# onolab-tmu/overiva

Measured on AMD Instinct MI355X. Metric: AuxIVA iterations/sec (2048 bins x 4000 frames x 8 mics), higher is better.
Workload: dtype f32

## Files before the change

include/overiva_hip.h:

```cpp
#ifndef OVERIVA_HIP_H
#define OVERIVA_HIP_H

#ifdef __cplusplus
extern "C" {
#endif

#define OIVA_OK 0
#define OIVA_ERR_ARG (-1)
#define OIVA_ERR_HIP (-2)
#define OIVA_ERR_STATE (-3)
#define OIVA_ERR_NUMERIC (-4)

#define OIVA_MODEL_LAPLACE 0
#define OIVA_MODEL_GAUSS 1

#define OIVA_MAX_CHANNELS 32

#define OIVA_PREC_FAST 0
#define OIVA_PREC_UPDATE_F64 1
#define OIVA_PREC_UPDATE_ROWS 2
#define OIVA_PREC_COV_F64 4
#define OIVA_PREC_PRECISE (OIVA_PREC_UPDATE_F64 | OIVA_PREC_COV_F64)

typedef struct oiva_plan oiva_plan;
// ... 47 lines not shown

int oiva_plan_sync(oiva_plan *p);
int oiva_plan_save_w(oiva_plan *p);
int oiva_plan_restore_w(oiva_plan *p);

int oiva_plan_iterate_timed(oiva_plan *p, int n, float *total_ms, float *per_kernel_ms);
#define OIVA_N_STAGES 4

int oiva_plan_get_cov_splits(oiva_plan *p, int *nsplit);
int oiva_plan_set_cov_splits(oiva_plan *p, int nsplit);
int oiva_plan_set_cov_quad(oiva_plan *p, int enable, int *active);
int oiva_plan_set_pow_splits(oiva_plan *p, int nsplit);
int oiva_plan_set_cov_hmfma(oiva_plan *p, int enable);
int oiva_plan_set_fuse_cov_update(oiva_plan *p, int enable, int *active);
int oiva_plan_set_power_reverse(oiva_plan *p, int enable);
int oiva_plan_set_x_resident_mb(oiva_plan *p, double mb);
int oiva_plan_get_x_resident(oiva_plan *p, int *n16, int *nt, int *reason);
int oiva_plan_use_graph(oiva_plan *p, int enable);
int oiva_plan_set_precision(oiva_plan *p, int flags);

struct oiva_xchg;
#define OIVA_RESIDENT_INFO 12
#define OIVA_RESIDENT_PHASES 8
int oiva_plan_set_resident(oiva_plan *p, int enable);
int oiva_plan_resident_info(oiva_plan *p, int *info );
int oiva_plan_resident_phases(oiva_plan *p, double *phase_us , int *n_iter);
int oiva_plan_resident_debug(oiva_plan *p, int timeout_ms, int stall_block);
int oiva_plan_resident_debug_from(oiva_plan *p, int timeout_ms, int stall_block, int first_stalled_iteration);
int oiva_plan_resident_loopback(oiva_plan *p, int world);
#define OIVA_RESIDENT_STAMPS 16
// ... 1 lines not shown
int oiva_plan_resident_connect(oiva_plan *p, struct oiva_xchg *x);
int oiva_plan_fused_connect(oiva_plan *p, struct oiva_xchg *x);
int oiva_plan_fused_loopback(oiva_plan *p, int world);
int oiva_plan_fused_debug(oiva_plan *p, int timeout_ms, int stall);
int oiva_plan_set_resident_splits(oiva_plan *p, int nsplit);

int oiva_test_set_rinv(oiva_plan *p, const float *rinv_host );
int oiva_test_get_rinv(oiva_plan *p, float *rinv_host , float *wscale_host );
int oiva_test_run_weighted_cov(oiva_plan *p);
int oiva_test_get_v(oiva_plan *p, void *V_host , int f64);
int oiva_test_run_update(oiva_plan *p);
int oiva_test_get_what(oiva_plan *p, void *What_host , int f64);
int oiva_test_set_what(oiva_plan *p, const void *What_host, int f64);
int oiva_test_run_power(oiva_plan *p, float *p_host );
int oiva_test_get_ppart(oiva_plan *p, float *parts_host, int *nparts);
int oiva_test_power_order(int nsplit, int tcp, int cov_splits, int cov_tc, int *order);
int oiva_test_time_stage(oiva_plan *p, int stage, int reps, float *avg_ms);
int oiva_test_live_buffers(long long *count, long long *bytes);
int oiva_test_x_policy(int T, int F, int M, int cov_tc, int pow_tcp, double budget_mb, int *out, signed char *cov_walk, signed char *pow_walk);
int oiva_test_x_choice(int T, int F, int M, int prec_flags, int cov_kind, int cov_tc, int pow_kind, int pow_tcp, double budget_mb, int from_env,
                       int *out, double *budget_used);
int oiva_test_kernel_choice(int device, int T, int F, int F_total, int M, int K, int prec_flags, int quad_on, int hmfma_on,
                            int cov_splits_req, int pow_splits_req, int *out);

#define OIVA_OGIVE_DEMIX 0
#define OIVA_OGIVE_MIX 1
#define OIVA_OGIVE_SWITCHING 2
int oiva_plan_ogive_begin(oiva_plan *p, int update_mode, int model);
int oiva_plan_ogive_iterate(oiva_plan *p, int first_epoch, int n, double step_size, double tol, int *epochs_run,
                            int *converged, double *max_delta);
// ... 114 lines not shown
```

overiva_amd/_lib.py:

```python
import ctypes as C
import os

import numpy as np

_PKG = os.path.dirname(os.path.abspath(__file__))
LIB_PATH = os.environ.get("OIVA_LIB") or os.path.join(_PKG, "liboveriva_hip.so")

OK, ERR_ARG, ERR_HIP, ERR_STATE, ERR_NUMERIC = 0, -1, -2, -3, -4
MODEL_IDS = {"laplace": 0, "gauss": 1}
N_STAGES = 4
PREC_FAST, PREC_UPDATE_F64, PREC_UPDATE_ROWS, PREC_COV_F64 = 0, 1, 2, 4
PREC_PRECISE = PREC_UPDATE_F64 | PREC_COV_F64
PREC_MIXED = PREC_UPDATE_F64
PREC_BY_NAME = {"fast": PREC_FAST, "mixed": PREC_MIXED, "precise": PREC_PRECISE}
STAGE_NAMES = ("demix_power", "activation", "weighted_cov", "ip_update")


class HipLibraryMissing(ImportError):
    pass


class HipError(RuntimeError):
    """a HIP runtime call failed inside the library"""

# ... 33 lines not shown
    "oiva_xchg_poll": [_vp, _i, _i, _vp],
    "oiva_xchg_force": [_vp, _i],
    "oiva_xchg_destroy": [_vp],
    "oiva_plan_get_w": [_vp, _vp, _i],
    "oiva_plan_sync": [_vp],
    "oiva_plan_save_w": [_vp],
    "oiva_plan_restore_w": [_vp],
    "oiva_plan_iterate_timed": [_vp, _i, _fp, _fp],
    "oiva_plan_get_cov_splits": [_vp, C.POINTER(_i)],
    "oiva_plan_set_cov_splits": [_vp, _i],
    "oiva_plan_set_cov_quad": [_vp, _i, C.POINTER(_i)],
    "oiva_plan_set_pow_splits": [_vp, _i],
    "oiva_plan_set_cov_hmfma": [_vp, _i],
    "oiva_plan_set_fuse_cov_update": [_vp, _i, C.POINTER(_i)],
    "oiva_plan_set_power_reverse": [_vp, _i],
    "oiva_plan_set_x_resident_mb": [_vp, C.c_double],
    "oiva_plan_get_x_resident": [_vp, C.POINTER(_i), C.POINTER(_i), C.POINTER(_i)],
    "oiva_plan_use_graph": [_vp, _i],
    "oiva_plan_set_precision": [_vp, _i],
    "oiva_plan_set_resident": [_vp, _i],
    "oiva_plan_resident_info": [_vp, C.POINTER(_i)],
    "oiva_plan_resident_phases": [_vp, C.POINTER(C.c_double), C.POINTER(_i)],
    "oiva_plan_resident_debug": [_vp, _i, _i],
    "oiva_plan_resident_debug_from": [_vp, _i, _i, _i],
    "oiva_plan_resident_loopback": [_vp, _i],
    "oiva_plan_fused_connect": [_vp, _vp],
    "oiva_plan_fused_loopback": [_vp, _i],
    "oiva_plan_fused_debug": [_vp, _i, _i],
    "oiva_plan_resident_connect": [_vp, _vp],
    "oiva_plan_resident_trace": [_vp, _i, _vp, C.POINTER(_i), C.POINTER(_i)],
    "oiva_plan_set_resident_splits": [_vp, _i],
    "oiva_test_set_rinv": [_vp, _vp],
    "oiva_test_get_rinv": [_vp, _vp, _vp],
    "oiva_test_run_weighted_cov": [_vp],
    "oiva_test_get_v": [_vp, _vp, _i],
    "oiva_test_run_update": [_vp],
    "oiva_test_get_what": [_vp, _vp, _i],
    "oiva_test_set_what": [_vp, _vp, _i],
    "oiva_test_run_power": [_vp, _vp],
    "oiva_test_get_ppart": [_vp, _vp, C.POINTER(_i)],
    "oiva_test_power_order": [_i, _i, _i, _i, C.POINTER(_i)],
    "oiva_test_x_choice": [_i] * 8 + [C.c_double, _i, C.POINTER(_i), C.POINTER(C.c_double)],
    "oiva_test_x_policy": [_i, _i, _i, _i, _i, C.c_double, C.POINTER(_i), _vp, _vp],
    "oiva_test_time_stage": [_vp, _i, _i, _fp],
    "oiva_test_live_buffers": [C.POINTER(C.c_longlong), C.POINTER(C.c_longlong)],
    "oiva_test_kernel_choice": [_i] * 11 + [C.POINTER(_i)],
    "oiva_plan_ogive_begin": [_vp, _i, _i],
    "oiva_plan_ogive_iterate": [_vp, _i, _i, C.c_double, C.c_double, C.POINTER(_i), C.POINTER(_i), C.POINTER(C.c_double)],
    "oiva_batch_create": [C.POINTER(_vp), _i, _i, _i, _i, _i, _i, _i, _vp],
    "oiva_batch_destroy": [_vp],
    "oiva_batch_set_x_host": [_vp, _vp, _i],
    "oiva_batch_set_x_dev": [_vp, _vp],
    "oiva_batch_covariance": [_vp],
    "oiva_batch_set_w": [_vp, _vp, _i],
    "oiva_batch_set_w_eig": [_vp],
# ... 177 lines not shown
```

overiva_amd/csrc/kernels_cov.hip:

```cpp

#include <cstdint>
#include <cstdlib>

#include "oiva_device.h"
#include "cov_arith.h"

namespace oiva {
namespace {

constexpr int kCovUnroll = 2;
constexpr int kChunk = 16;
constexpr int kLdsStride = kBlock + 1;

template <int M, int KC, typename ACC, typename At>
__device__ __forceinline__ void reduce_and_store_at(At&& at, ACC* lds, double* __restrict__ Vpart, int F, int K, int k0) {
    constexpr int NA = M * M;
    constexpr int NACC = NA * KC;
    const int tid = threadIdx.x;
    const int bb = tid >> 4, aa = tid & 15;
    const int fo = blockIdx.x * kBinsPerWave + bb;
    double* out = Vpart + (((size_t)blockIdx.y * F + fo) * K + k0) * NA;
#pragma unroll
    for (int r0 = 0; r0 < NACC; r0 += kChunk) {
        __syncthreads();
// ... 3 lines not shown
        }
        __syncthreads();
        double s = 0.;
#pragma unroll
        for (int qq = 0; qq < 16; ++qq) s += (double)lds[aa * kLdsStride + qq * 16 + bb];
        const int e = r0 + aa;
        const int kk = e / NA;
        if (e < NACC && fo < F && k0 + kk < K) out[e] = s;
    }
}

template <int M, int KC, typename ACC>
__device__ __forceinline__ void reduce_and_store(const ACC (&acc)[KC][M * M], ACC* lds, double* __restrict__ Vpart,
                                                 int F, int K, int k0) {
    reduce_and_store_at<M, KC, ACC>([&](int e) { return acc[e / (M * M)][e % (M * M)]; }, lds, Vpart, F, K, k0);
}

template <int M, int KC, bool UNIT, typename ACC>
__global__ __launch_bounds__(kBlock) void cov_kernel(const float2* __restrict__ X, const float* __restrict__ R,
                                                     float* __restrict__ wscale, int model, int raw,
                                                     double* __restrict__ Vpart, int T, int F, int K, int tc, int ) {
    constexpr int NA = M * M;
    __shared__ ACC lds[kChunk * kLdsStride];

    const int tid = threadIdx.x;
    const int lane = tid & 63;
    const int wave = tid >> 6;
    const int b = lane & (kBinsPerWave - 1);
    const int q = wave * kPhasesPerWave + (lane >> 4);
    const int f = blockIdx.x * kBinsPerWave + b;
// ... 73 lines not shown

constexpr int kDmaStages = 4;

#ifdef OIVA_COVDMA_TRACE
__device__ long long g_cd_trace[8 * 2048];
#define CD_STAMP(slot)                                                                                                            \
    do {                                                                                                                          \
        if (threadIdx.x == 0 && blockIdx.z == 0) g_cd_trace[(blockIdx.y * gridDim.x + blockIdx.x) * 8 + (slot)] = wall_clock64(); \
    } while (0)
#else
#define CD_STAMP(slot) \
    do {               \
    } while (0)
#endif

template <int M, int KC>
__global__ __launch_bounds__(kBlock, 2) void cov_dma_kernel(const float2* __restrict__ X, const float* __restrict__ R,
                                                            float* __restrict__ wscale, int model, int raw,
                                                            double* __restrict__ Vpart, int T, int F, int K, int tc, int xplain) {
    constexpr int NA = M * M;
    constexpr int PIECES = M / 2;
    constexpr int STAGE = PIECES * 64;
    static_assert(M % 2 == 0 && (PIECES == 2 || PIECES == 4), "LDS-DMA path: M in {4, 8}");
    __shared__ float4 ring[kWaves * kDmaStages * STAGE];
    static_assert(sizeof(float4) * kWaves * kDmaStages * STAGE >= sizeof(float) * kChunk * kLdsStride,
                  "reduction scratch aliases the ring");

    const int tid = threadIdx.x;
    const int lane = tid & 63;
    const int wave = __builtin_amdgcn_readfirstlane(tid >> 6);
    const int b = lane & (kBinsPerWave - 1);
// ... 72 lines not shown
            }
            pacc.add(x, v2f{w[0], w[1]});
        } else {
            float xr[M], xi[M];
#pragma unroll
            for (int j = 0; j < PIECES; ++j) {
                xr[2 * j] = v[j].x;
                xi[2 * j] = v[j].y;
                xr[2 * j + 1] = v[j].z;
                xi[2 * j + 1] = v[j].w;
            }
            accumulate<M, KC, false, float>(acc, xr, xi, w);
        }
    };

    CD_STAMP(0);
    issue(0, 0);
    issue(1, 1);
    issue(2, 2);
#pragma unroll
    for (int kk = 0; kk < KC; ++kk) {
        const int k = k0 + kk;
        ginv[kk] = 1.f;
        if (raw & 1) continue;
#if defined(OIVA_COVDMA_ABLATE) && (OIVA_COVDMA_ABLATE & 4)
        const float gamma = R[k < K ? k : K - 1] + 1.f;
#else
        const float gamma = (float)gamma_of(R, T, K, k < K ? k : K - 1);
#endif
        ginv[kk] = 1.f / gamma;
        if (blockIdx.x == 0 && blockIdx.y == 0 && threadIdx.x == 0 && k < K && wscale != nullptr)
            wscale[k] = model == OIVA_MODEL_LAPLACE ? gamma : sqrtf(gamma);
    }

    CD_STAMP(1);
    int i = 0;
    for (; i + 4 <= nsteps; i += 4) {
        issue(i + 3, 3); consume(i, 0);
        issue(i + 4, 0); consume(i + 1, 1);
        issue(i + 5, 1); consume(i + 2, 2);
        issue(i + 6, 2); consume(i + 3, 3);
    }
    if (i < nsteps) { issue(i + 3, 3); consume(i, 0); }
    if (i + 1 < nsteps) { issue(i + 4, 0); consume(i + 1, 1); }
    if (i + 2 < nsteps) { issue(i + 5, 1); consume(i + 2, 2); }
    CD_STAMP(2);
    asm volatile("s_waitcnt vmcnt(0)" ::: "memory");
    CD_STAMP(3);
#if defined(OIVA_COVDMA_ABLATE) && (OIVA_COVDMA_ABLATE & 2)
    if constexpr (kPacked) {
        if (pacc.at(0) == 12345.f) Vpart[0] = 1.;
        return;
    }
#endif
    if constexpr (kPacked)
        reduce_and_store_at<M, KC, float>([&](int e) { return pacc.at(e); }, reinterpret_cast<float*>(ring), Vpart, F, K, k0);
    else
        reduce_and_store<M, KC, float>(acc, reinterpret_cast<float*>(ring), Vpart, F, K, k0);
    CD_STAMP(4);
}

template <typename ACC>
using CovKernel = void (*)(const float2*, const float*, float*, int, int, double*, int, int, int, int, int);

template <int M, typename ACC, typename Fn>
hipError_t dispatch_kc(int kc, bool unit, Fn&& fn) {
    constexpr int kRegs = M * M * (int)(sizeof(ACC) / 4);
    if (unit) return kc == 1 ? fn((CovKernel<ACC>)cov_kernel<M, 1, true, ACC>, 1) : hipErrorInvalidValue;
    if constexpr ((M == 4 || M == 8) && sizeof(ACC) == 4) {
        switch (kc) {
            case 1:
                return fn((CovKernel<ACC>)cov_dma_kernel<M, 1>, 1);
            case 2:
                if constexpr (kRegs * 2 <= 144) return fn((CovKernel<ACC>)cov_dma_kernel<M, 2>, 2);
                break;
            case 4:
                if constexpr (kRegs * 4 <= 144) return fn((CovKernel<ACC>)cov_dma_kernel<M, 4>, 4);
                break;
        }
        return hipErrorInvalidValue;
    }
    switch (kc) {
        case 1:
            return fn((CovKernel<ACC>)cov_kernel<M, 1, false, ACC>, 1);
        case 2:
            if constexpr (kRegs * 2 <= 144) return fn((CovKernel<ACC>)cov_kernel<M, 2, false, ACC>, 2);
            break;
        case 4:
            if constexpr (kRegs * 4 <= 144) return fn((CovKernel<ACC>)cov_kernel<M, 4, false, ACC>, 4);
            break;
        case 3:
            if constexpr (M == 7 && sizeof(ACC) == 4) return fn((CovKernel<ACC>)cov_kernel<M, 3, false, ACC>, 3);
            break;
        case 5:
            if constexpr (M == 5 && sizeof(ACC) == 4) return fn((CovKernel<ACC>)cov_kernel<M, 5, false, ACC>, 5);
            break;
    }
    return hipErrorInvalidValue;
}

template <typename ACC, typename Fn>
hipError_t dispatch_cov(int M, int kc, bool unit, Fn&& fn) {
    switch (M) {
        case 1: return dispatch_kc<1, ACC>(kc, unit, fn);
        case 2: return dispatch_kc<2, ACC>(kc, unit, fn);
        case 3: return dispatch_kc<3, ACC>(kc, unit, fn);
        case 4: return dispatch_kc<4, ACC>(kc, unit, fn);
        case 5: return dispatch_kc<5, ACC>(kc, unit, fn);
        case 6: return dispatch_kc<6, ACC>(kc, unit, fn);
        case 7: return dispatch_kc<7, ACC>(kc, unit, fn);
        case 8: return dispatch_kc<8, ACC>(kc, unit, fn);
    }
    return hipErrorInvalidValue;
}

}

__global__ __launch_bounds__(kBlock) void pad_channels_kernel(const float2* __restrict__ X, float2* __restrict__ Xpad, long long n, int M) {
    const long long e = (long long)blockIdx.x * kBlock + threadIdx.x;
    if (e >= n) return;
    const long long tf = e / (M + 1);
    const int c = (int)(e - tf * (M + 1));
    Xpad[e] = c < M ? X[tf * M + c] : make_float2(0.f, 0.f);
}

hipError_t launch_pad_channels(hipStream_t s, const float2* X, float2* Xpad, long long n_tf, int M) {
    const long long n = n_tf * (M + 1);
    pad_channels_kernel<<<dim3((unsigned)((n + kBlock - 1) / kBlock)), dim3(kBlock), 0, s>>>(X, Xpad, n, M);
    return hipGetLastError();
}

hipError_t launch_cov(hipStream_t s, const float2* X, const float2* Xpad, const float* R, float* Wt, float* wscale, int model, int raw,
                      void* Vpart, bool f64, int T, int F, int M, int K, const CovGeom& g) {
    const CovTraits& t = traits(g.kind);
    if (g.tc % t.quantum != 0 || (g.pad && Xpad == nullptr)) return hipErrorInvalidValue;
    const float2* Xv = g.pad && t.padded_x ? Xpad : X;
    const int Mp = g.pad && t.padded_x ? M + 1 : M;
    double* const V64 = static_cast<double*>(Vpart);
    switch (g.kind) {
        case CovKind::Wide: return launch_cov_wide(s, X, R, Wt, wscale, model, raw, V64, T, F, M, K, g);
        case CovKind::Half16: return launch_cov_half16(s, Xv, R, Wt, wscale, model, raw, V64, T, F, Mp, M, K, g);
        case CovKind::Hmfma: {
            const hipError_t e = launch_cov_half16_weights(s, R, Wt, wscale, model, raw, T, K);
            return e != hipSuccess ? e : launch_cov_hmfma(s, Xv, Wt, V64, T, F, Mp, M, K, g);
        }
        case CovKind::Half16F64: return launch_cov_half16_f64(s, Xv, R, Wt, wscale, model, raw, V64, T, F, Mp, M, K, g);
        case CovKind::Hmfma64: {
            const hipError_t e = launch_cov_half16_weights_f64(s, R, Wt, wscale, model, raw, T, K);
            return e != hipSuccess ? e : launch_cov_hmfma64(s, Xv, reinterpret_cast<const double*>(Wt), V64, T, F, Mp, M, K, g);
        }
        case CovKind::Quad: return launch_cov_quad(s, Xv, R, Wt, wscale, model, raw, V64, T, F, Mp, M, K, g);
        case CovKind::Mfma: return launch_cov_mfma(s, X, R, Wt, wscale, model, raw, Vpart, f64, T, F, M, K, g.nsplit, g.tc);
        case CovKind::Pair32: return launch_cov_pair32(s, X, R, Wt, wscale, model, raw, V64, T, F, M, K, g);
        case CovKind::Pair64: return launch_cov_pair64(s, X, R, Wt, wscale, model, raw, V64, T, F, M, K, g);
        case CovKind::Lane: break;
    }
    const int kc = R == nullptr ? 1 : g.kc;
    if (f64)
        return dispatch_cov<double>(M, kc, R == nullptr, [&](CovKernel<double> kern, int KC) {
            kern<<<dim3(g.nbg, g.nsplit, (K + KC - 1) / KC), dim3(kBlock), 0, s>>>(X, R, wscale, model, raw,
                                                                                 static_cast<double*>(Vpart), T, F, K, g.tc, g.xplain);
            return hipGetLastError();
        });
    return dispatch_cov<float>(M, kc, R == nullptr, [&](CovKernel<float> kern, int KC) {
        return launch_dominant(kern, dim3(g.nbg, g.nsplit, (K + KC - 1) / KC), dim3(kBlock), 0, s, X, R, wscale, model, raw,
                               static_cast<double*>(Vpart), T, F, K, g.tc, g.xplain);
    });
}

hipError_t cov_blocks_per_cu(int M, int kc, bool f64, int* n) {
    if (f64)
        return dispatch_cov<double>(M, kc, false, [&](CovKernel<double> kern, int) {
            return hipOccupancyMaxActiveBlocksPerMultiprocessor(n, kern, kBlock, 0);
        });
    return dispatch_cov<float>(M, kc, false, [&](CovKernel<float> kern, int) {
        return hipOccupancyMaxActiveBlocksPerMultiprocessor(n, kern, kBlock, 0);
    });
}

#ifdef OIVA_COVDMA_TRACE
extern "C" int oiva_debug_covdma_trace(long long* out) { return (int)hipMemcpyFromSymbol(out, HIP_SYMBOL(g_cd_trace), sizeof(g_cd_trace)); }
#endif

}
```

overiva_amd/csrc/oiva_internal.h:

```cpp
#pragma once
#include <hip/hip_runtime.h>
#include <hip/hip_ext.h>

#include <string>

#include "kernel_choice.h"
#include "overiva_hip.h"

namespace oiva {

int fail_with(int code, const std::string& msg);
int xchg_peers(oiva_xchg* x, char** peers, int* rank, int* world, size_t* slot_bytes);

__host__ __device__ inline int herm_pair_index(int M, int c, int d) {
    return M + 2 * (c * M - (c * (c + 1)) / 2 + (d - c - 1));
}

__host__ __device__ inline size_t rsum_offset_floats(int T, int K) { return (((size_t)T + kPhasesPerWave) * K + 1) & ~(size_t)1; }
__host__ __device__ inline int rsum_blocks(int T) { return (T + kBlock - 1) / kBlock; }
__host__ __device__ inline size_t r_buffer_bytes(int T, int K) {
    return rsum_offset_floats(T, K) * sizeof(float) + (size_t)rsum_blocks(T) * K * sizeof(double);
}

struct KernelTimer {
// ... 14 lines not shown
        hipLaunchKernelGGL(kernel, grid, block, shmem, s, args...);
    }
    return hipGetLastError();
}

__host__ __device__ inline int power_chunk_tail_first(int y, int n, const PowOrder& o) {
    if (y < o.q * o.cs) return o.first[y % o.cs + 1] - 1 - y / o.cs;
    y -= o.q * o.cs;
    for (int r = o.q; r < n; ++r)
        for (int s = 0; s < o.cs; ++s)
            if (o.first[s + 1] - o.first[s] > r && y-- == 0) return o.first[s + 1] - 1 - r;
    return n - 1;
}

hipError_t launch_cov(hipStream_t s, const float2* X, const float2* Xpad, const float* R, float* Wt, float* wscale, int model, int raw,
                      void* Vpart, bool f64, int T, int F, int M, int K, const CovGeom& g);
hipError_t launch_pad_channels(hipStream_t s, const float2* X, float2* Xpad, long long n_tf, int M);
hipError_t launch_cov_mfma(hipStream_t s, const float2* X, const float* R, float* Wt, float* wscale, int model, int raw,
                           void* Vpart, bool f64, int T, int F, int M, int K, int nsplit, int tc);
hipError_t launch_cov_quad(hipStream_t s, const float2* X, const float* R, float* Wt, float* wscale, int model, int raw,
                           double* Vpart, int T, int F, int M, int Mv, int K, const CovGeom& g);
hipError_t launch_cov_weights(hipStream_t s, const float* R, float* Wt, float* wscale, int model, int raw, int T, int K, int Kp);
hipError_t launch_cov_pair64(hipStream_t s, const float2* X, const float* R, float* Wt, float* wscale, int model, int raw,
                             double* Vpart, int T, int F, int M, int K, const CovGeom& g);
hipError_t launch_cov_pair32(hipStream_t s, const float2* X, const float* R, float* Wt, float* wscale, int model, int raw,
                             double* Vpart, int T, int F, int M, int K, const CovGeom& g);
hipError_t launch_cov_half16(hipStream_t s, const float2* X, const float* R, float* Wt, float* wscale, int model, int raw,
                             double* Vpart, int T, int F, int M, int Mv, int K, const CovGeom& g);
hipError_t launch_cov_half16_weights(hipStream_t s, const float* R, float* Wt, float* wscale, int model, int raw, int T, int K);
hipError_t launch_cov_half16_weights_f64(hipStream_t s, const float* R, float* Wt, float* wscale, int model, int raw, int T, int K);
hipError_t launch_cov_hmfma(hipStream_t s, const float2* X, const float* Wt, double* Vpart, int T, int F, int M, int Mv, int K, const CovGeom& g);
// ... 314 lines not shown
```

overiva_amd/csrc/plan.hip:

```cpp
#include <algorithm>
#include <cmath>
#include <cstdint>
#include <cstdlib>
#include <cstring>
#include <mutex>
#include <string>
#include <vector>

#include "host_io.h"
#include "host_util.h"
#include "oiva_internal.h"
#include "resident.h"

using namespace oiva;

namespace {

constexpr int kGraphBatch = 8;
constexpr int kGraphMaxIters = 32;
constexpr int kGraphCache = 6;

}

struct oiva_plan {
// ... 13 lines not shown
    float* Ppart = nullptr;
    int ppart_alloc = 0;
    float* Plocal = nullptr;
    void* Wwide = nullptr;
    float* R = nullptr;
    float* wscale = nullptr;
    float* Spart = nullptr;
    float2* Y = nullptr;
    double2* scratch_c = nullptr;
    double* scratch_p = nullptr;

    CovGeom cov{};
    bool cov_quad_on = true;
    bool cov_hmfma_on = true;
    bool fuse_cov_update = false;
    int power_reverse = 1;
    int pow_splits_req = 0;
    double x_resident_mb = kXResidentDefaultMB;
    CovGeom stg{};
    PowGeom pw{};
    int n_cu = 256;
    int vpart_splits_alloc = 0;

    bool have_x = false, have_cx = false, have_w = false;
    bool pad_valid = false;
    bool wscale_pending = false;
    int raw_weights = 0;
    int prec = 0;
    bool upd_f64() const { return prec & OIVA_PREC_UPDATE_F64; }
    bool cov_f64() const { return prec & OIVA_PREC_COV_F64; }
// ... 140 lines not shown
}
int stage_activation(oiva_plan* p, const float* parts, int nparts) {
    if (p->fx_on && parts == p->Ppart) {
        OIVA_TRY_HIP(launch_activation_xchg(p->stream, parts, nparts, p->fx_gath, p->fx_rank, p->fx_world, p->fx_loopback ? (p->fx_stall ? 2 : 1) : 0, p->fx_nblk_own, p->fx_nblk_peer, p->fx_state + 16,
                                       p->fx_state, (long long)(p->fx_timeout_ms > 0 ? p->fx_timeout_ms : 2000) * 100000, p->R, p->T, p->K,
                                       p->model, p->F_total));
        p->raw_weights = 0;
        return OIVA_OK;
    }
    OIVA_TRY_HIP(launch_activation(p->stream, parts, nparts, p->R, p->T, p->K, p->model, p->F_total));
    p->raw_weights = 0;
    return OIVA_OK;
}
int stage_cov(oiva_plan* p) {
    OIVA_TRY_HIP(launch_cov(p->stream, p->X, p->X_pad, p->R, p->Wwide ? static_cast<float*>(p->Wwide) : p->Plocal , p->wscale, p->model,
                       p->raw_weights, p->Vpart, p->cov_f64(), p->T, p->F, p->M, p->K, cov_geom_now(p)));
    p->wscale_pending = !p->raw_weights;
    return OIVA_OK;
}
int stage_update(oiva_plan* p, bool init_only) {
    UpdateArgs a;
    a.What = p->What;
    a.What64 = p->upd_f64() ? p->What64 : nullptr;
    a.Cx = p->Cx;
    a.Vpart = p->Vpart;
    a.vpart_f64 = p->vpart_f64() ? 1 : 0;
    a.wscale = (!init_only && p->wscale_pending) ? p->wscale : nullptr;
    a.nsplit = p->cov.nsplit;
    a.T = p->T;
    a.F = p->F;
    a.M = p->M;
// ... 280 lines not shown
        if (hipGetDeviceProperties(&prop, device) == hipSuccess && prop.multiProcessorCount > 0)
            p->n_cu = prop.multiProcessorCount;
    }
    if (M > 8 && M <= kNarrowMax && M % 2 == 1) {
        const hipError_t ep = p->mem.take_one(&p->X_pad, (size_t)T * F * (M + 1) * sizeof(float2));
        if (ep != hipSuccess) {
            oiva_plan_destroy(p);
            return fail_with(OIVA_ERR_HIP, std::string("allocation of the padded copy of X failed: ") + hipGetErrorString(ep));
        }
    }
    {
        const char* v = std::getenv("OIVA_COV_HMFMA");
        p->cov_hmfma_on = !(v && v[0] == '0');
        const char* u = std::getenv("OIVA_COV_UPDATE");
        p->fuse_cov_update = u && u[0] == '1';
        const char* r = std::getenv("OIVA_POWER_REVERSE");
        p->power_reverse = (r && r[0] == '0') ? 0 : (r && r[0] == '2') ? 2 : 1;
        const char* x = std::getenv("OIVA_X_RESIDENT_MB");
        if (x && x[0]) p->x_resident_mb = std::atof(x);
    }
    choose_cov_geom(p, 0);
    choose_pow_geom(p, 0);
    choose_stats_geom(p);
    p->res_ok = resident_geometry(T, F, M, K, p->n_cu, 0, &p->rg);
    const size_t nTK = (size_t)T * K;
    const size_t nFMM = (size_t)F * M * M;
    DeviceArena& mem = p->mem;
    mem.take(&p->What, nFMM * sizeof(float2));
    mem.take(&p->What64, nFMM * sizeof(double2));
    mem.take(&p->Cx, nFMM * sizeof(double));
// ... 579 lines not shown
    OIVA_NEED(p, OIVA_ERR_ARG, "null plan");
    return change_geometry(p, [&] { p->cov_hmfma_on = enable != 0; choose_cov_geom(p, 0); return OIVA_OK; });
}

int oiva_plan_set_pow_splits(oiva_plan* p, int nsplit) {
    OIVA_NEED(p, OIVA_ERR_ARG, "null plan");
    OIVA_NEED(nsplit >= 0 && nsplit <= p->T, OIVA_ERR_ARG, "bad split count");
    return change_geometry(p, [&] { choose_pow_geom(p, nsplit); return OIVA_OK; });
}

int oiva_plan_set_power_reverse(oiva_plan* p, int enable) {
    OIVA_NEED(p, OIVA_ERR_ARG, "null plan");
    return change_geometry(p, [&] { p->power_reverse = enable < 0 ? 0 : enable > 2 ? 2 : enable; return OIVA_OK; });
}

int oiva_plan_set_x_resident_mb(oiva_plan* p, double mb) {
    OIVA_NEED(p, OIVA_ERR_ARG, "null plan");
    OIVA_NEED(mb == mb, OIVA_ERR_ARG, "the budget is not a number");
    return change_geometry(p, [&] { p->x_resident_mb = mb; choose_pow_geom(p, p->pow_splits_req); return OIVA_OK; });
}

int oiva_plan_get_x_resident(oiva_plan* p, int* n16, int* nt, int* reason) {
    OIVA_NEED(p && n16 && nt && reason, OIVA_ERR_ARG, "null argument");
    const XPolicy x = x_policy(p);
    *n16 = x.n16, *nt = x.nt ? 1 : 0, *reason = (int)x.why;
    return OIVA_OK;
}

int oiva_plan_use_graph(oiva_plan* p, int enable) {
    OIVA_NEED(p, OIVA_ERR_ARG, "null plan");
// ... 207 lines not shown
    if (rc) return rc;
    OIVA_NEED(p->og_ready, OIVA_ERR_STATE, "call oiva_plan_ogive_begin first");
    OIVA_NEED(n >= 0 && first_epoch >= 0, OIVA_ERR_ARG, "negative epoch count");
    DeviceGuard guard(p->device);
    int before[2] = {0, 0};
    OIVA_TRY_HIP(hipStreamSynchronize(p->stream));
    OIVA_TRY_HIP(hipMemcpy(before, p->og.ctrl, sizeof(before), hipMemcpyDeviceToHost));
    const int amodel = p->og_model == OIVA_MODEL_LAPLACE ? kModelOgiveLaplace : OIVA_MODEL_GAUSS;
    auto epochs = [&](int e0, int count) -> int {
        for (int e = e0; e < e0 + count; ++e) {
            if (p->og_mode == OIVA_OGIVE_SWITCHING && e % 10 == 0) OIVA_TRY_HIP(launch_ogive_switch(p->stream, p->og, p->F, p->M));
            int r = stage_power(p);
            if (r) return r;
            OIVA_TRY_HIP(launch_activation(p->stream, p->Ppart, p->pw.nb, p->R, p->T, 1, amodel, p->F));
            OIVA_TRY_HIP(launch_cov(p->stream, p->X, p->X_pad, p->R, p->Plocal, p->wscale, p->model,  1, p->Vpart,
                               p->cov_f64(), p->T, p->F, p->M, 1, cov_geom_now(p)));
            OIVA_TRY_HIP(launch_ogive_step(p->stream, p->og, p->Vpart, p->vpart_f64(), p->cov.nsplit, p->T, p->F, p->M, step_size,
                                      tol));
        }
        return OIVA_OK;
    };
    constexpr int kMinGraphEpochs = 8;
    if (n >= kMinGraphEpochs) {
        const int phase = first_epoch % 10;
        if (!p->og_graph || p->og_graph_n != n || p->og_graph_phase != phase || p->og_graph_mu != step_size ||
            p->og_graph_tol != tol) {
            if (p->og_graph) OIVA_TRY_HIP(hipGraphExecDestroy(p->og_graph));
            p->og_graph = nullptr;
            rc = capture_graph(p->stream, [&] { return epochs(phase, n); }, &p->og_graph, false);
            if (rc) return rc;
            p->og_graph_n = n;
// ... 154 lines not shown
    OIVA_TRY_HIP(hipMemcpy(sum.data(), p->scratch_p, n * sizeof(double), hipMemcpyDeviceToHost));
    for (size_t i = 0; i < n; ++i) p_host[i] = (float)sum[i];
    return OIVA_OK;
}

int oiva_test_get_ppart(oiva_plan* p, float* parts_host, int* nparts) {
    OIVA_NEED(p && nparts, OIVA_ERR_ARG, "null argument");
    *nparts = p->pw.nb;
    if (!parts_host) return OIVA_OK;
    DeviceGuard guard(p->device);
    OIVA_TRY_HIP(hipStreamSynchronize(p->stream));
    OIVA_TRY_HIP(hipMemcpy(parts_host, p->Ppart, (size_t)p->pw.nb * p->T * p->K * sizeof(float), hipMemcpyDeviceToHost));
    return OIVA_OK;
}

int oiva_test_power_order(int nsplit, int tcp, int cov_splits, int cov_tc, int* order) {
    OIVA_NEED(order && nsplit >= 1 && tcp >= 1 && cov_splits >= 1 && cov_tc >= 1, OIVA_ERR_ARG, "bad arguments");
    OIVA_NEED(cov_splits <= kPowOrderMaxSplits, OIVA_ERR_ARG, "more covariance splits than the order table holds");
    const PowOrder o = make_pow_order(nsplit, tcp, cov_splits, cov_tc);
    for (int y = 0; y < nsplit; ++y) order[y] = power_chunk_tail_first(y, nsplit, o);
    return OIVA_OK;
}

int oiva_test_x_policy(int T, int F, int M, int cov_tc, int pow_tcp, double budget_mb, int* out, signed char* cov_walk, signed char* pow_walk) {
    OIVA_NEED(out && cov_walk && pow_walk && T >= 1 && F >= 1 && M >= 1 && cov_tc >= 1 && pow_tcp >= 1, OIVA_ERR_ARG, "bad arguments");
    CovGeom cg{};
    cg.tc = cov_tc, cg.nsplit = ceil_div(T, cov_tc);
    PowGeom pg{};
    pg.tcp = pow_tcp, pg.nsplit = ceil_div(T, pow_tcp);
    const XPolicy x = choose_x_policy(budget_mb, T, F, M, false, cg, pg);
// ... 58 lines not shown
```

overiva_amd/plan.py:

```python
import ctypes as C

import numpy as np

from . import _lib


def _is_f64(a):
    if a.dtype == np.complex128:
        return 1
    if a.dtype == np.complex64:
        return 0
    raise TypeError(f"complex64 or complex128 expected, got {a.dtype}")


class DeviceX:

    def __init__(self, ptr, shape, owner=None, host_dtype=np.complex64):
        self.ptr = int(ptr)
        self.shape = tuple(int(v) for v in shape)
        self.owner = owner
        self.dtype = np.dtype(host_dtype)
        self.ndim = 3


# ... 153 lines not shown

    def set_cov_hmfma(self, enable=True):
        _lib.check(self.lib.oiva_plan_set_cov_hmfma(self.h, 1 if enable else 0))

    def set_fuse_cov_update(self, enable=True):
        a = C.c_int()
        _lib.check(self.lib.oiva_plan_set_fuse_cov_update(self.h, -1 if enable is None else (1 if enable else 0), C.byref(a)))
        return bool(a.value)

    def set_pow_splits(self, n):
        _lib.check(self.lib.oiva_plan_set_pow_splits(self.h, int(n)))

    def set_power_reverse(self, enable=True):
        _lib.check(self.lib.oiva_plan_set_power_reverse(self.h, int(enable)))

    X_RESIDENT_REASONS = ("off", "fits", "kernels", "geometry", "share")

    def set_x_resident_mb(self, mb):
        _lib.check(self.lib.oiva_plan_set_x_resident_mb(self.h, float(mb)))

    def x_resident(self):
        n16, nt, why = C.c_int(), C.c_int(), C.c_int()
        _lib.check(self.lib.oiva_plan_get_x_resident(self.h, C.byref(n16), C.byref(nt), C.byref(why)))
        return n16.value, bool(nt.value), self.X_RESIDENT_REASONS[why.value]

    def use_graph(self, enable=True):
        _lib.check(self.lib.oiva_plan_use_graph(self.h, 1 if enable else 0))

    def set_precision(self, mode="fast", row_layout=False):
        flags = _lib.PREC_BY_NAME[mode] if isinstance(mode, str) else int(mode)
# ... 80 lines not shown
        What = np.asarray(What)
        What = np.ascontiguousarray(What, dtype=np.complex64 if What.dtype == np.complex64 else np.complex128)
        assert What.shape == (self.F, self.M, self.M)
        _lib.check(self.lib.oiva_test_set_what(self.h, _lib.ptr(What), _is_f64(What)))

    def t_time_stage(self, stage, reps=20):
        ms = C.c_float()
        _lib.check(self.lib.oiva_test_time_stage(self.h, _lib.STAGE_NAMES.index(stage), int(reps), C.byref(ms)))
        return ms.value

    def t_get_ppart(self):
        n = C.c_int()
        _lib.check(self.lib.oiva_test_get_ppart(self.h, None, C.byref(n)))
        out = np.empty((n.value, self.T, self.K), np.float32)
        _lib.check(self.lib.oiva_test_get_ppart(self.h, _lib.ptr(out), C.byref(n)))
        return out

    def t_run_power(self):
        p = np.empty((self.T, self.K), np.float32)
        _lib.check(self.lib.oiva_test_run_power(self.h, _lib.ptr(p)))
        return p


COV_KINDS = ("Lane", "Pair32", "Pair64", "Quad", "Half16", "Hmfma", "Half16F64", "Hmfma64", "Mfma", "Wide")
POW_KINDS = ("Lane", "Mfma", "Lds", "Wide")
KERNEL_CHOICE = ("cov_kind", "nsplit", "tc", "kc", "nbg", "pad", "part32", "vpart_f64", "unit_kind", "pow_kind", "nb", "pow_nsplit",
                 "tcp", "kp", "rounds", "occ_cov", "occ_pow", "n_cu")


def kernel_choice(T, F, M, K, mode="fast", F_total=None, cov_quad=True, cov_hmfma=True, cov_splits=0, pow_splits=0, device=0,
# ... 13 lines not shown
```

Before: 5651.

## Skip out-of-range DMA prefetches and vectorize cov epilogue reduction

Adds a SHORT_TAIL variant of the covariance DMA kernel, on by default. It stops issuing prefetches past the last time step and waits only for the loads it needs (counted vmcnt) instead of running past the end. For M=8 packed accumulators it also adds a float4-vectorized, XOR-swizzled LDS reduction epilogue that writes double2 stores. The intent is to cut wasted loads and waits at the pipeline tail and speed up the final reduction, at the cost of more template instantiations and tighter vmcnt bookkeeping.

```diff
diff --git a/include/overiva_hip.h b/include/overiva_hip.h
--- a/include/overiva_hip.h
+++ b/include/overiva_hip.h
@@ -85,6 +85,7 @@
 int oiva_plan_set_cov_hmfma(oiva_plan *p, int enable);
 int oiva_plan_set_fuse_cov_update(oiva_plan *p, int enable, int *active);
 int oiva_plan_set_power_reverse(oiva_plan *p, int enable);
+int oiva_plan_set_cov_tail(oiva_plan *p, int enable);
 int oiva_plan_set_x_resident_mb(oiva_plan *p, double mb);
 int oiva_plan_get_x_resident(oiva_plan *p, int *n16, int *nt, int *reason);
 int oiva_plan_use_graph(oiva_plan *p, int enable);
@@ -116,6 +117,7 @@
 int oiva_test_set_what(oiva_plan *p, const void *What_host, int f64);
 int oiva_test_run_power(oiva_plan *p, float *p_host );
 int oiva_test_get_ppart(oiva_plan *p, float *parts_host, int *nparts);
+int oiva_test_get_vpart(oiva_plan *p, double *parts_host, int *nsplit);
 int oiva_test_power_order(int nsplit, int tcp, int cov_splits, int cov_tc, int *order);
 int oiva_test_time_stage(oiva_plan *p, int stage, int reps, float *avg_ms);
 int oiva_test_live_buffers(long long *count, long long *bytes);
diff --git a/overiva_amd/_lib.py b/overiva_amd/_lib.py
--- a/overiva_amd/_lib.py
+++ b/overiva_amd/_lib.py
@@ -71,6 +71,7 @@
     "oiva_plan_set_cov_hmfma": [_vp, _i],
     "oiva_plan_set_fuse_cov_update": [_vp, _i, C.POINTER(_i)],
     "oiva_plan_set_power_reverse": [_vp, _i],
+    "oiva_plan_set_cov_tail": [_vp, _i],
     "oiva_plan_set_x_resident_mb": [_vp, C.c_double],
     "oiva_plan_get_x_resident": [_vp, C.POINTER(_i), C.POINTER(_i), C.POINTER(_i)],
     "oiva_plan_use_graph": [_vp, _i],
@@ -96,6 +97,7 @@
     "oiva_test_set_what": [_vp, _vp, _i],
     "oiva_test_run_power": [_vp, _vp],
     "oiva_test_get_ppart": [_vp, _vp, C.POINTER(_i)],
+    "oiva_test_get_vpart": [_vp, _vp, C.POINTER(_i)],
     "oiva_test_power_order": [_i, _i, _i, _i, C.POINTER(_i)],
     "oiva_test_x_choice": [_i] * 8 + [C.c_double, _i, C.POINTER(_i), C.POINTER(C.c_double)],
     "oiva_test_x_policy": [_i, _i, _i, _i, _i, C.c_double, C.POINTER(_i), _vp, _vp],
diff --git a/overiva_amd/csrc/kernels_cov.hip b/overiva_amd/csrc/kernels_cov.hip
--- a/overiva_amd/csrc/kernels_cov.hip
+++ b/overiva_amd/csrc/kernels_cov.hip
@@ -41,6 +41,39 @@
 __device__ __forceinline__ void reduce_and_store(const ACC (&acc)[KC][M * M], ACC* lds, double* __restrict__ Vpart,
                                                  int F, int K, int k0) {
     reduce_and_store_at<M, KC, ACC>([&](int e) { return acc[e / (M * M)][e % (M * M)]; }, lds, Vpart, F, K, k0);
+}
+
+template <typename At>
+__device__ __forceinline__ void reduce_and_store_vec(At&& at, float4* lds, double* __restrict__ Vpart, int F, int K, int k0) {
+    constexpr int NA = 64;
+    const int tid = threadIdx.x;
+    const int bb = tid >> 4, aa = tid & 15;
+    const int fo = blockIdx.x * kBinsPerWave + bb;
+    double2* out = reinterpret_cast<double2*>(Vpart + (((size_t)blockIdx.y * F + fo) * K + k0) * NA + 4 * aa);
+    float4* wr = lds + tid * 16;
+    const int wx = tid & 7;
+    const float4* rd = lds + bb * 16 + (aa ^ (bb & 7));
+#pragma unroll
+    for (int r = 0; r < 2; ++r) {
+        __syncthreads();
+#pragma unroll
+        for (int j = 0; j < 16; ++j)
+            wr[j ^ wx] = make_float4(at(NA * r + 4 * j), at(NA * r + 4 * j + 1), at(NA * r + 4 * j + 2), at(NA * r + 4 * j + 3));
+        __syncthreads();
+        double s0 = 0., s1 = 0., s2 = 0., s3 = 0.;
+#pragma unroll
+        for (int qq = 0; qq < 16; ++qq) {
+            const float4 v = rd[qq * 256];
+            s0 += (double)v.x;
+            s1 += (double)v.y;
+            s2 += (double)v.z;
+            s3 += (double)v.w;
+        }
+        if (fo < F && k0 + r < K) {
+            out[r * (NA / 2)] = make_double2(s0, s1);
+            out[r * (NA / 2) + 1] = make_double2(s2, s3);
+        }
+    }
 }
 
 template <int M, int KC, bool UNIT, typename ACC>
@@ -144,7 +177,7 @@
     } while (0)
 #endif
 
-template <int M, int KC>
+template <int M, int KC, bool SHORT_TAIL>
 __global__ __launch_bounds__(kBlock, 2) void cov_dma_kernel(const float2* __restrict__ X, const float* __restrict__ R,
                                                             float* __restrict__ wscale, int model, int raw,
                                                             double* __restrict__ Vpart, int T, int F, int K, int tc, int xplain) {
@@ -247,10 +280,20 @@
         }
     };
 
+    auto wait_behind = [&](int behind) {
+        if (behind >= kDmaStages - 1) return;
+        if (behind == 2)
+            asm volatile("s_waitcnt vmcnt(%0)" ::"n"(2 * PIECES) : "memory");
+        else if (behind == 1)
+            asm volatile("s_waitcnt vmcnt(%0)" ::"n"(PIECES) : "memory");
+        else
+            asm volatile("s_waitcnt vmcnt(0)" ::: "memory");
+    };
+
     CD_STAMP(0);
     issue(0, 0);
-    issue(1, 1);
-    issue(2, 2);
+    if (!SHORT_TAIL || 1 < nsteps) issue(1, 1);
+    if (!SHORT_TAIL || 2 < nsteps) issue(2, 2);
 #pragma unroll
     for (int kk = 0; kk < KC; ++kk) {
         const int k = k0 + kk;
@@ -268,15 +311,30 @@
 
     CD_STAMP(1);
     int i = 0;
-    for (; i + 4 <= nsteps; i += 4) {
-        issue(i + 3, 3); consume(i, 0);
-        issue(i + 4, 0); consume(i + 1, 1);
-        issue(i + 5, 1); consume(i + 2, 2);
-        issue(i + 6, 2); consume(i + 3, 3);
-    }
-    if (i < nsteps) { issue(i + 3, 3); consume(i, 0); }
-    if (i + 1 < nsteps) { issue(i + 4, 0); consume(i + 1, 1); }
-    if (i + 2 < nsteps) { issue(i + 5, 1); consume(i + 2, 2); }
+    if constexpr (SHORT_TAIL) {
+        auto ahead = [&](int j, int s) {
+            if (j < nsteps) issue(j, s);
+        };
+        for (; i + 4 <= nsteps; i += 4) {
+            ahead(i + 3, 3); wait_behind(nsteps - 1 - i); consume(i, 0);
+            ahead(i + 4, 0); wait_behind(nsteps - 2 - i); consume(i + 1, 1);
+            ahead(i + 5, 1); wait_behind(nsteps - 3 - i); consume(i + 2, 2);
+            ahead(i + 6, 2); wait_behind(nsteps - 4 - i); consume(i + 3, 3);
+        }
+        if (i < nsteps) { wait_behind(nsteps - 1 - i); consume(i, 0); }
+        if (i + 1 < nsteps) { wait_behind(nsteps - 2 - i); consume(i + 1, 1); }
+        if (i + 2 < nsteps) { wait_behind(0); consume(i + 2, 2); }
+    } else {
+        for (; i + 4 <= nsteps; i += 4) {
+            issue(i + 3, 3); consume(i, 0);
+            issue(i + 4, 0); consume(i + 1, 1);
+            issue(i + 5, 1); consume(i + 2, 2);
+            issue(i + 6, 2); consume(i + 3, 3);
+        }
+        if (i < nsteps) { issue(i + 3, 3); consume(i, 0); }
+        if (i + 1 < nsteps) { issue(i + 4, 0); consume(i + 1, 1); }
+        if (i + 2 < nsteps) { issue(i + 5, 1); consume(i + 2, 2); }
+    }
     CD_STAMP(2);
     asm volatile("s_waitcnt vmcnt(0)" ::: "memory");
     CD_STAMP(3);
@@ -286,7 +344,15 @@
         return;
     }
 #endif
-    if constexpr (kPacked)
+#if defined(OIVA_COVDMA_ABLATE) && (OIVA_COVDMA_ABLATE & 8)
+    constexpr bool kVecEpilogue = false;
+#else
+    constexpr bool kVecEpilogue = kPacked && M == 8 && SHORT_TAIL;
+#endif
+    if constexpr (kVecEpilogue) {
+        static_assert(sizeof(ring) >= kBlock * 64 * sizeof(float), "reduce_and_store_vec's image fits the ring");
+        reduce_and_store_vec([&](int e) { return pacc.at(e); }, ring, Vpart, F, K, k0);
+    } else if constexpr (kPacked)
         reduce_and_store_at<M, KC, float>([&](int e) { return pacc.at(e); }, reinterpret_cast<float*>(ring), Vpart, F, K, k0);
     else
         reduce_and_store<M, KC, float>(acc, reinterpret_cast<float*>(ring), Vpart, F, K, k0);
@@ -297,18 +363,18 @@
 using CovKernel = void (*)(const float2*, const float*, float*, int, int, double*, int, int, int, int, int);
 
 template <int M, typename ACC, typename Fn>
-hipError_t dispatch_kc(int kc, bool unit, Fn&& fn) {
+hipError_t dispatch_kc(int kc, bool unit, bool short_tail, Fn&& fn) {
     constexpr int kRegs = M * M * (int)(sizeof(ACC) / 4);
     if (unit) return kc == 1 ? fn((CovKernel<ACC>)cov_kernel<M, 1, true, ACC>, 1) : hipErrorInvalidValue;
     if constexpr ((M == 4 || M == 8) && sizeof(ACC) == 4) {
         switch (kc) {
             case 1:
-                return fn((CovKernel<ACC>)cov_dma_kernel<M, 1>, 1);
+                return fn(short_tail ? (CovKernel<ACC>)cov_dma_kernel<M, 1, true> : (CovKernel<ACC>)cov_dma_kernel<M, 1, false>, 1);
             case 2:
-                if constexpr (kRegs * 2 <= 144) return fn((CovKernel<ACC>)cov_dma_kernel<M, 2>, 2);
+                if constexpr (kRegs * 2 <= 144) return fn(short_tail ? (CovKernel<ACC>)cov_dma_kernel<M, 2, true> : (CovKernel<ACC>)cov_dma_kernel<M, 2, false>, 2);
                 break;
             case 4:
-                if constexpr (kRegs * 4 <= 144) return fn((CovKernel<ACC>)cov_dma_kernel<M, 4>, 4);
+                if constexpr (kRegs * 4 <= 144) return fn(short_tail ? (CovKernel<ACC>)cov_dma_kernel<M, 4, true> : (CovKernel<ACC>)cov_dma_kernel<M, 4, false>, 4);
                 break;
         }
         return hipErrorInvalidValue;
@@ -333,16 +399,16 @@
 }
 
 template <typename ACC, typename Fn>
-hipError_t dispatch_cov(int M, int kc, bool unit, Fn&& fn) {
+hipError_t dispatch_cov(int M, int kc, bool unit, bool short_tail, Fn&& fn) {
     switch (M) {
-        case 1: return dispatch_kc<1, ACC>(kc, unit, fn);
-        case 2: return dispatch_kc<2, ACC>(kc, unit, fn);
-        case 3: return dispatch_kc<3, ACC>(kc, unit, fn);
-        case 4: return dispatch_kc<4, ACC>(kc, unit, fn);
-        case 5: return dispatch_kc<5, ACC>(kc, unit, fn);
-        case 6: return dispatch_kc<6, ACC>(kc, unit, fn);
-        case 7: return dispatch_kc<7, ACC>(kc, unit, fn);
-        case 8: return dispatch_kc<8, ACC>(kc, unit, fn);
+        case 1: return dispatch_kc<1, ACC>(kc, unit, short_tail, fn);
+        case 2: return dispatch_kc<2, ACC>(kc, unit, short_tail, fn);
+        case 3: return dispatch_kc<3, ACC>(kc, unit, short_tail, fn);
+        case 4: return dispatch_kc<4, ACC>(kc, unit, short_tail, fn);
+        case 5: return dispatch_kc<5, ACC>(kc, unit, short_tail, fn);
+        case 6: return dispatch_kc<6, ACC>(kc, unit, short_tail, fn);
+        case 7: return dispatch_kc<7, ACC>(kc, unit, short_tail, fn);
+        case 8: return dispatch_kc<8, ACC>(kc, unit, short_tail, fn);
     }
     return hipErrorInvalidValue;
 }
@@ -364,7 +430,7 @@
 }
 
 hipError_t launch_cov(hipStream_t s, const float2* X, const float2* Xpad, const float* R, float* Wt, float* wscale, int model, int raw,
-                      void* Vpart, bool f64, int T, int F, int M, int K, const CovGeom& g) {
+                      void* Vpart, bool f64, int T, int F, int M, int K, const CovGeom& g, bool short_tail) {
     const CovTraits& t = traits(g.kind);
     if (g.tc % t.quantum != 0 || (g.pad && Xpad == nullptr)) return hipErrorInvalidValue;
     const float2* Xv = g.pad && t.padded_x ? Xpad : X;
@@ -390,12 +456,12 @@
     }
     const int kc = R == nullptr ? 1 : g.kc;
     if (f64)
-        return dispatch_cov<double>(M, kc, R == nullptr, [&](CovKernel<double> kern, int KC) {
+        return dispatch_cov<double>(M, kc, R == nullptr, short_tail, [&](CovKernel<double> kern, int KC) {
             kern<<<dim3(g.nbg, g.nsplit, (K + KC - 1) / KC), dim3(kBlock), 0, s>>>(X, R, wscale, model, raw,
                                                                                  static_cast<double*>(Vpart), T, F, K, g.tc, g.xplain);
             return hipGetLastError();
         });
-    return dispatch_cov<float>(M, kc, R == nullptr, [&](CovKernel<float> kern, int KC) {
+    return dispatch_cov<float>(M, kc, R == nullptr, short_tail, [&](CovKernel<float> kern, int KC) {
         return launch_dominant(kern, dim3(g.nbg, g.nsplit, (K + KC - 1) / KC), dim3(kBlock), 0, s, X, R, wscale, model, raw,
                                static_cast<double*>(Vpart), T, F, K, g.tc, g.xplain);
     });
@@ -403,10 +469,10 @@
 
 hipError_t cov_blocks_per_cu(int M, int kc, bool f64, int* n) {
     if (f64)
-        return dispatch_cov<double>(M, kc, false, [&](CovKernel<double> kern, int) {
+        return dispatch_cov<double>(M, kc, false, true, [&](CovKernel<double> kern, int) {
             return hipOccupancyMaxActiveBlocksPerMultiprocessor(n, kern, kBlock, 0);
         });
-    return dispatch_cov<float>(M, kc, false, [&](CovKernel<float> kern, int) {
+    return dispatch_cov<float>(M, kc, false, true, [&](CovKernel<float> kern, int) {
         return hipOccupancyMaxActiveBlocksPerMultiprocessor(n, kern, kBlock, 0);
     });
 }
diff --git a/overiva_amd/csrc/oiva_internal.h b/overiva_amd/csrc/oiva_internal.h
--- a/overiva_amd/csrc/oiva_internal.h
+++ b/overiva_amd/csrc/oiva_internal.h
@@ -52,7 +52,7 @@
 }
 
 hipError_t launch_cov(hipStream_t s, const float2* X, const float2* Xpad, const float* R, float* Wt, float* wscale, int model, int raw,
-                      void* Vpart, bool f64, int T, int F, int M, int K, const CovGeom& g);
+                      void* Vpart, bool f64, int T, int F, int M, int K, const CovGeom& g, bool short_tail = true);
 hipError_t launch_pad_channels(hipStream_t s, const float2* X, float2* Xpad, long long n_tf, int M);
 hipError_t launch_cov_mfma(hipStream_t s, const float2* X, const float* R, float* Wt, float* wscale, int model, int raw,
                            void* Vpart, bool f64, int T, int F, int M, int K, int nsplit, int tc);
diff --git a/overiva_amd/csrc/plan.hip b/overiva_amd/csrc/plan.hip
--- a/overiva_amd/csrc/plan.hip
+++ b/overiva_amd/csrc/plan.hip
@@ -51,6 +51,7 @@
     bool cov_quad_on = true;
     bool cov_hmfma_on = true;
     bool fuse_cov_update = false;
+    int cov_tail = 1;
     int power_reverse = 1;
     int pow_splits_req = 0;
     double x_resident_mb = kXResidentDefaultMB;
@@ -221,7 +222,7 @@
 }
 int stage_cov(oiva_plan* p) {
     OIVA_TRY_HIP(launch_cov(p->stream, p->X, p->X_pad, p->R, p->Wwide ? static_cast<float*>(p->Wwide) : p->Plocal , p->wscale, p->model,
-                       p->raw_weights, p->Vpart, p->cov_f64(), p->T, p->F, p->M, p->K, cov_geom_now(p)));
+                       p->raw_weights, p->Vpart, p->cov_f64(), p->T, p->F, p->M, p->K, cov_geom_now(p), p->cov_tail != 0));
     p->wscale_pending = !p->raw_weights;
     return OIVA_OK;
 }
@@ -532,6 +533,8 @@
         p->cov_hmfma_on = !(v && v[0] == '0');
         const char* u = std::getenv("OIVA_COV_UPDATE");
         p->fuse_cov_update = u && u[0] == '1';
+        const char* ct = std::getenv("OIVA_COV_TAIL");
+        p->cov_tail = (ct && ct[0] == '0') ? 0 : 1;
         const char* r = std::getenv("OIVA_POWER_REVERSE");
         p->power_reverse = (r && r[0] == '0') ? 0 : (r && r[0] == '2') ? 2 : 1;
         const char* x = std::getenv("OIVA_X_RESIDENT_MB");
@@ -1141,6 +1144,11 @@
     return change_geometry(p, [&] { p->power_reverse = enable < 0 ? 0 : enable > 2 ? 2 : enable; return OIVA_OK; });
 }
 
+int oiva_plan_set_cov_tail(oiva_plan* p, int enable) {
+    OIVA_NEED(p, OIVA_ERR_ARG, "null plan");
+    return change_geometry(p, [&] { p->cov_tail = enable != 0; return OIVA_OK; });
+}
+
 int oiva_plan_set_x_resident_mb(oiva_plan* p, double mb) {
     OIVA_NEED(p, OIVA_ERR_ARG, "null plan");
     OIVA_NEED(mb == mb, OIVA_ERR_ARG, "the budget is not a number");
@@ -1378,7 +1386,7 @@
             if (r) return r;
             OIVA_TRY_HIP(launch_activation(p->stream, p->Ppart, p->pw.nb, p->R, p->T, 1, amodel, p->F));
             OIVA_TRY_HIP(launch_cov(p->stream, p->X, p->X_pad, p->R, p->Plocal, p->wscale, p->model,  1, p->Vpart,
-                               p->cov_f64(), p->T, p->F, p->M, 1, cov_geom_now(p)));
+                               p->cov_f64(), p->T, p->F, p->M, 1, cov_geom_now(p), p->cov_tail != 0));
             OIVA_TRY_HIP(launch_ogive_step(p->stream, p->og, p->Vpart, p->vpart_f64(), p->cov.nsplit, p->T, p->F, p->M, step_size,
                                       tol));
         }
@@ -1563,6 +1571,17 @@
     return OIVA_OK;
 }
 
+int oiva_test_get_vpart(oiva_plan* p, double* parts_host, int* nsplit) {
+    OIVA_NEED(p && nsplit, OIVA_ERR_ARG, "null argument");
+    OIVA_NEED(p->vpart_f64(), OIVA_ERR_STATE, "the partial covariances of this plan are not float64");
+    *nsplit = p->cov.nsplit;
+    if (!parts_host) return OIVA_OK;
+    DeviceGuard guard(p->device);
+    OIVA_TRY_HIP(hipStreamSynchronize(p->stream));
+    OIVA_TRY_HIP(hipMemcpy(parts_host, p->Vpart, vpart_floats(p, p->cov.nsplit) * sizeof(double), hipMemcpyDeviceToHost));
+    return OIVA_OK;
+}
+
 int oiva_test_power_order(int nsplit, int tcp, int cov_splits, int cov_tc, int* order) {
     OIVA_NEED(order && nsplit >= 1 && tcp >= 1 && cov_splits >= 1 && cov_tc >= 1, OIVA_ERR_ARG, "bad arguments");
     OIVA_NEED(cov_splits <= kPowOrderMaxSplits, OIVA_ERR_ARG, "more covariance splits than the order table holds");
diff --git a/overiva_amd/plan.py b/overiva_amd/plan.py
--- a/overiva_amd/plan.py
+++ b/overiva_amd/plan.py
@@ -191,6 +191,9 @@
     def set_power_reverse(self, enable=True):
         _lib.check(self.lib.oiva_plan_set_power_reverse(self.h, int(enable)))
 
+    def set_cov_tail(self, enable=True):
+        _lib.check(self.lib.oiva_plan_set_cov_tail(self.h, 1 if enable else 0))
+
     X_RESIDENT_REASONS = ("off", "fits", "kernels", "geometry", "share")
 
     def set_x_resident_mb(self, mb):
@@ -301,6 +304,13 @@
         _lib.check(self.lib.oiva_test_get_ppart(self.h, None, C.byref(n)))
         out = np.empty((n.value, self.T, self.K), np.float32)
         _lib.check(self.lib.oiva_test_get_ppart(self.h, _lib.ptr(out), C.byref(n)))
+        return out
+
+    def t_get_vpart(self):
+        n = C.c_int()
+        _lib.check(self.lib.oiva_test_get_vpart(self.h, None, C.byref(n)))
+        out = np.empty((n.value, self.F, self.K, self.M * self.M), np.float64)
+        _lib.check(self.lib.oiva_test_get_vpart(self.h, _lib.ptr(out), C.byref(n)))
         return out
 
     def t_run_power(self):
```

After: 5680, median of 3. Within noise of the previous version (+0.5%).
